# frasermince/gym-cellular-automata

Measured on AMD Instinct MI355X. Metric: cell-updates/sec, 4096x(256x256) ForestFireBulldozer (Alexandridis CA), per-GPU batch, higher is better.
Workload: dtype u8 cells / i16 ages / f32 probabilities

## Files before the change

gym-cellular-automata_amd/csrc/gca_alex_march.hip:

```cpp
#include "gca_alex_rule.h"

#include <type_traits>

#ifndef GCA_MARCH_FLAT_OCC
#define GCA_MARCH_FLAT_OCC 4
#endif
#ifndef GCA_MARCH_OBS_FLAT_OCC
#define GCA_MARCH_OBS_FLAT_OCC 3
#endif
#ifndef GCA_MARCH_XROW
#define GCA_MARCH_XROW 1
#endif

namespace {

constexpr int MW = 256;
constexpr int SH = 16;

struct MarchObs {
    const float4* col;
    const int32_t* night;
    float* rgb;
    const int32_t* action;
    int action_stride, n_choices;
    uint32_t mode_bits;
    uint8_t* refit;
};
constexpr uint32_t OBS_GRID = 0u, OBS_ZERO = 1u, OBS_NONE = 2u;
constexpr uint32_t OBS_CHK_GRID = 4u, OBS_CHK_BLUR = 8u;

__device__ __forceinline__ uint32_t from_prev(uint32_t v) {
    return (uint32_t)__builtin_amdgcn_mov_dpp((int)v, 0x138, 0xF, 0xF, true);
}
__device__ __forceinline__ uint32_t from_next(uint32_t v) {
    return (uint32_t)__builtin_amdgcn_mov_dpp((int)v, 0x130, 0xF, 0xF, true);
}
__device__ __forceinline__ uint32_t from_prev_or(uint32_t old, uint32_t v) {
    return (uint32_t)__builtin_amdgcn_update_dpp((int)old, (int)v, 0x138, 0xF, 0xF, false);
}
__device__ __forceinline__ uint32_t from_next_or(uint32_t old, uint32_t v) {
    return (uint32_t)__builtin_amdgcn_update_dpp((int)old, (int)v, 0x130, 0xF, 0xF, false);
}

template <int J> __device__ __forceinline__ uint64_t byte_lanes(uint32_t x) {
    static_assert(J >= 0 && J < 4, "byte 0..3");
    uint64_t m;
    const uint32_t zero = 0u;
    if constexpr (J == 0) asm("v_cmp_ne_u32_sdwa %0, %1, %2 src0_sel:BYTE_0 src1_sel:DWORD" : "=s"(m) : "v"(x), "s"(zero));
    if constexpr (J == 1) asm("v_cmp_ne_u32_sdwa %0, %1, %2 src0_sel:BYTE_1 src1_sel:DWORD" : "=s"(m) : "v"(x), "s"(zero));
    if constexpr (J == 2) asm("v_cmp_ne_u32_sdwa %0, %1, %2 src0_sel:BYTE_2 src1_sel:DWORD" : "=s"(m) : "v"(x), "s"(zero));
    if constexpr (J == 3) asm("v_cmp_ne_u32_sdwa %0, %1, %2 src0_sel:BYTE_3 src1_sel:DWORD" : "=s"(m) : "v"(x), "s"(zero));
    return m;
}
__device__ __forceinline__ uint32_t lanes_select(uint32_t c, uint64_t m) {
    uint32_t o;
    asm("v_cndmask_b32_e64 %0, 0, %1, %2" : "=v"(o) : "v"(c), "s"(m));
    return o;
}

__host__ __device__ constexpr uint32_t win_mask(int o, int j, int k) {
    uint32_t m = 0;
    for (int b = 0; b < 4; ++b) {
        const int c = 4 * o + b - j;
        if (c >= -k && c <= k) m |= 1u << (8 * b);
    }
    return m;
}
__host__ __device__ constexpr bool win_full(int o, int j, int k) { return j - k <= 4 * o && 4 * o + 3 <= j + k; }
template <bool HALO = false>
__device__ __forceinline__ void window4(uint32_t X, int k, uint32_t (&B)[4], uint32_t z = 0u, uint32_t h1 = 0u,
                                        uint32_t h2 = 0u) {
    uint32_t n[5] = {0u, 0u, X, 0u, 0u};
    if (k >= 1) {
        n[1] = HALO ? from_prev_or(h1, X) : from_prev(X);
        n[3] = HALO ? from_next_or(h1, X) : from_next(X);
    }
    if (k >= 5) {
        n[0] = HALO ? from_prev_or(h2, n[1]) : from_prev(n[1]);
        n[4] = HALO ? from_next_or(h2, n[3]) : from_next(n[3]);
    }
    constexpr uint32_t ONES = 0x01010101u;
    bool use0 = false, useL = false, useR = false, useLR = false;
#pragma unroll
    for (int j = 0; j < 4; ++j) {
        const bool f0 = win_full(0, j, k), fl = win_full(-1, j, k), fr = win_full(1, j, k);
        if (f0 && fl && fr) useLR = true;
        else if (f0 && fl) useL = true;
        else if (f0 && fr) useR = true;
        else if (f0) use0 = true;
    }
    uint32_t S0 = 0u, SL = 0u, SR = 0u, SLR = 0u;
    if (use0 || useL || useR || useLR) S0 = __builtin_amdgcn_udot4(n[2], ONES, z, false);
    if (useL || useLR) SL = __builtin_amdgcn_udot4(n[1], ONES, S0, false);
    if (useR) SR = __builtin_amdgcn_udot4(n[3], ONES, S0, false);
    if (useLR) SLR = __builtin_amdgcn_udot4(n[3], ONES, SL, false);
#pragma unroll
    for (int j = 0; j < 4; ++j) {
        const bool f0 = win_full(0, j, k), fl = win_full(-1, j, k), fr = win_full(1, j, k);
        const bool run = f0;
        uint32_t acc = !run ? z : (fl && fr) ? SLR : fl ? SL : fr ? SR : S0;
#pragma unroll
        for (int o = -2; o <= 2; ++o) {
            if (run && (o == 0 || (o == -1 && fl) || (o == 1 && fr))) continue;
            const uint32_t m = win_mask(o, j, k);
            if (m) acc = __builtin_amdgcn_udot4(n[o + 2], m, acc, false);
        }
        B[j] = acc;
    }
}

__device__ __forceinline__ float4 ldf4(const float* p) { return *reinterpret_cast<const float4*>(p); }
__device__ __forceinline__ gca_f2 m_recip(float v0, float v1) {
    const gca_f2 x = {v0, v1};
    const gca_f2 r0 = {__builtin_amdgcn_rcpf(v0), __builtin_amdgcn_rcpf(v1)};
    const gca_f2 ee = __builtin_elementwise_fma(-x, r0, (gca_f2){1.0f, 1.0f});
    return __builtin_elementwise_fma(ee, r0, r0);
}
__device__ __forceinline__ void m_edge_both(float v0, float v1, gca_f2& own, gca_f2& nb) {
    const gca_f2 rc = m_recip(v0, v1);
    asm("v_max_f32_e64 %0, %1, -%2" : "=v"(own.x) : "v"(v0), "v"(rc.x));
    asm("v_max_f32_e64 %0, %1, -%2" : "=v"(own.y) : "v"(v1), "v"(rc.y));
    asm("v_max_f32_e64 %0, -%1, %2" : "=v"(nb.x) : "v"(v0), "v"(rc.x));
    asm("v_max_f32_e64 %0, -%1, %2" : "=v"(nb.y) : "v"(v1), "v"(rc.y));
}
__device__ __forceinline__ void m_edge_both4(const float4& v, gca_f2& oa, gca_f2& na, gca_f2& ob, gca_f2& nb) {
    const gca_f2 x0 = {v.x, v.y}, x1 = {v.z, v.w};
    const gca_f2 r0 = {__builtin_amdgcn_rcpf(v.x), __builtin_amdgcn_rcpf(v.y)};
    const gca_f2 r1 = {__builtin_amdgcn_rcpf(v.z), __builtin_amdgcn_rcpf(v.w)};
    const gca_f2 e0 = __builtin_elementwise_fma(-x0, r0, (gca_f2){1.0f, 1.0f});
    const gca_f2 e1 = __builtin_elementwise_fma(-x1, r1, (gca_f2){1.0f, 1.0f});
    const gca_f2 c0 = __builtin_elementwise_fma(e0, r0, r0);
    const gca_f2 c1 = __builtin_elementwise_fma(e1, r1, r1);
    asm("v_max_f32_e64 %0, %1, -%2" : "=v"(oa.x) : "v"(v.x), "v"(c0.x));
    asm("v_max_f32_e64 %0, %1, -%2" : "=v"(oa.y) : "v"(v.y), "v"(c0.y));
    asm("v_max_f32_e64 %0, %1, -%2" : "=v"(ob.x) : "v"(v.z), "v"(c1.x));
    asm("v_max_f32_e64 %0, %1, -%2" : "=v"(ob.y) : "v"(v.w), "v"(c1.y));
    asm("v_max_f32_e64 %0, -%1, %2" : "=v"(na.x) : "v"(v.x), "v"(c0.x));
    asm("v_max_f32_e64 %0, -%1, %2" : "=v"(na.y) : "v"(v.y), "v"(c0.y));
    asm("v_max_f32_e64 %0, -%1, %2" : "=v"(nb.x) : "v"(v.z), "v"(c1.x));
    asm("v_max_f32_e64 %0, -%1, %2" : "=v"(nb.y) : "v"(v.w), "v"(c1.y));
}
__device__ __forceinline__ void m_edge_own4(const float4& v, gca_f2& oa, gca_f2& ob) {
    const gca_f2 x0 = {v.x, v.y}, x1 = {v.z, v.w};
    const gca_f2 r0 = {__builtin_amdgcn_rcpf(v.x), __builtin_amdgcn_rcpf(v.y)};
    const gca_f2 r1 = {__builtin_amdgcn_rcpf(v.z), __builtin_amdgcn_rcpf(v.w)};
    const gca_f2 e0 = __builtin_elementwise_fma(-x0, r0, (gca_f2){1.0f, 1.0f});
    const gca_f2 e1 = __builtin_elementwise_fma(-x1, r1, (gca_f2){1.0f, 1.0f});
    const gca_f2 c0 = __builtin_elementwise_fma(e0, r0, r0);
    const gca_f2 c1 = __builtin_elementwise_fma(e1, r1, r1);
    asm("v_max_f32_e64 %0, %1, -%2" : "=v"(oa.x) : "v"(v.x), "v"(c0.x));
    asm("v_max_f32_e64 %0, %1, -%2" : "=v"(oa.y) : "v"(v.y), "v"(c0.y));
    asm("v_max_f32_e64 %0, %1, -%2" : "=v"(ob.x) : "v"(v.z), "v"(c1.x));
    asm("v_max_f32_e64 %0, %1, -%2" : "=v"(ob.y) : "v"(v.w), "v"(c1.y));
}
template <class T, class B> __device__ __forceinline__ T ld_at(const B* base, uint32_t off) {
    return *reinterpret_cast<const T*>(reinterpret_cast<const unsigned char*>(base) + off);
}
template <class T, class B> __device__ __forceinline__ T ld_nt(const B* base, uint32_t off) {
    constexpr int N = (int)(sizeof(T) / 4);
    typedef uint32_t vt __attribute__((ext_vector_type(N)));
    typedef const __attribute__((address_space(1))) unsigned char gbyte;
    typedef const __attribute__((address_space(1))) vt gvt;
    const vt v = __builtin_nontemporal_load((gvt*)((gbyte*)base + off));
    return __builtin_bit_cast(T, v);
}
constexpr uint32_t WZ = 0x4B000000u;
__device__ __forceinline__ gca_f2 wsum_f2(uint32_t b0, uint32_t b1) {
    return (gca_f2){__uint_as_float(b0), __uint_as_float(b1)} - (gca_f2){8388608.0f, 8388608.0f};
}
typedef uint16_t u16x2 __attribute__((ext_vector_type(2)));
typedef int16_t i16x2 __attribute__((ext_vector_type(2)));
__device__ __forceinline__ i16x2 bitcast_i16x2(uint32_t v) { return __builtin_bit_cast(i16x2, v); }
__device__ __forceinline__ u16x2 bitcast_u16x2(uint32_t v) { return __builtin_bit_cast(u16x2, v); }
template <class T> __device__ __forceinline__ uint32_t bitcast_u32(T v) { return __builtin_bit_cast(uint32_t, v); }

constexpr int XI = 16;
constexpr int XS_ONE = 13, XS_TWO = 14;

template <int R, bool OBS, bool GROW, int NSEG, int FLATM>
__global__ __launch_bounds__(NSEG == 1 ? 256 : 64 * NSEG) __attribute__((amdgpu_waves_per_eu(OBS ? (FLATM ? GCA_MARCH_OBS_FLAT_OCC : 2) : (FLATM ? GCA_MARCH_FLAT_OCC : 3), OBS ? (FLATM ? GCA_MARCH_OBS_FLAT_OCC : 2) : (FLATM ? GCA_MARCH_FLAT_OCC : 3)))) void alex_march_kernel(
    gca_alex_params p, int H, int nwaves, const uint8_t* __restrict__ grid_in, uint8_t* __restrict__ grid_out,
    const int16_t* age_in, int16_t* age_out,
    const uint8_t* __restrict__ vd, const uint16_t* __restrict__ dbits, const float* __restrict__ es,
    const int32_t* __restrict__ wind_index, const uint32_t* __restrict__ rng_step, int32_t* __restrict__ counts,
    const uint8_t* __restrict__ act_in, uint8_t* __restrict__ act_out, MarchObs obs) {
    constexpr int NF = 2 * R + 1;
    constexpr int RB = R;
    constexpr bool HALO = NSEG > 1;
    constexpr bool SMASK = !HALO && !OBS && FLATM >= 1;
    constexpr int WPB = HALO ? NSEG : 4;
    constexpr int W = MW * NSEG;
    __shared__ float lut[WPB][16];
    __shared__ float4 colw[WPB][8];
    __shared__ float4 img[OBS ? WPB : 1][OBS ? 192 : 1];
    __shared__ uint32_t fring[WPB][2 * NF * 64];
    __shared__ uint32_t xch[HALO ? 2 : 1][HALO ? NSEG + 2 : 1][4][HALO ? XI : 1];
    __shared__ uint32_t qfl[HALO ? NSEG : 1];
    constexpr bool FLAT = FLATM >= 1, UNI = FLATM == 2;
    constexpr bool XROW = GCA_MARCH_XROW && !HALO && OBS && !FLAT;
    __shared__ float4 xrow[XROW ? 4 : 1][3][XROW ? 64 : 1];
    __shared__ uint32_t xok[XROW ? 4 : 1];

    const int tid = threadIdx.x, wl = __builtin_amdgcn_readfirstlane(tid >> 6), lane = tid & 63;
    const int nb = (int)gridDim.x;
    const int xcd = (int)blockIdx.x & 7, slot = (int)blockIdx.x >> 3;
    const int qn8 = nb >> 3, rn8 = nb & 7;
    const int lb = (xcd < rn8 ? xcd * (qn8 + 1) : rn8 * (qn8 + 1) + (xcd - rn8) * qn8) + slot;
    int strips, e, s, g;
    if constexpr (!HALO) {
        const int wv = lb * 4 + wl;
        if (wv >= nwaves) {
            if constexpr (XROW) {
                if (lane == 0) xok[wl] = 0u;
                __builtin_amdgcn_fence(__ATOMIC_RELEASE, "workgroup", "local");
                __builtin_amdgcn_s_barrier();
            }
            return;
        }
        strips = H / SH;
        e = wv / strips;
        s = wv - e * strips;
        g = 0;
    } else {
        if (lb * NSEG >= nwaves) return;
        strips = H / SH;
        e = lb / strips;
        s = lb - e * strips;
        g = wl;
    }
    const int s0 = s * SH;
    const uint32_t HW = (uint32_t)H * W;
    const uint8_t* gE = grid_in + (size_t)e * HW;
    uint8_t* gO = grid_out + (size_t)e * HW;
    const int16_t* aE = age_in + (size_t)e * HW;
    int16_t* aO = age_out + (size_t)e * HW;
    const uint8_t* vE = UNI ? vd : vd + (size_t)e * HW;
    const uint16_t* dE = dbits + (size_t)e * (HW >> 4);
    const float* sE = FLAT ? es : es + (size_t)e * 4 * HW;
    const uint32_t lc = HALO ? (uint32_t)(MW * g) + 4u * (uint32_t)lane : 4u * (uint32_t)lane;
    const uint32_t ld16 = HALO ? lc >> 4 : (uint32_t)(lane >> 2);
    const uint32_t lane_a = 2u * lc, lane_s = 4u * lc, lane_d = 2u * ld16;
    const uint32_t Fp = rep4((uint32_t)p.fire), Ep = rep4((uint32_t)p.empty), Tp = rep4((uint32_t)p.tree);

    if (lane < 16) lut[wl][lane] = gca_alex_lut_entry(p, lane);
    if (OBS && lane < 6) colw[wl][lane] = obs.col[6 * (obs.night[e] != 0 ? 1 : 0) + lane];
    uint32_t omode = 0u;
    if constexpr (OBS && !HALO) {
        if (obs.action) {
            const int choice = min(max(obs.action[(size_t)e * obs.action_stride + 2], 0), obs.n_choices - 1);
            omode = (uint32_t)__builtin_amdgcn_readfirstlane((int)((obs.mode_bits >> (4 * choice)) & 0xFu));
        }
    }
    auto row0_refit = [&](uint32_t x0, uint32_t x1) -> uint8_t {
        const uint32_t odd = ((x0 + 0x7D7D7D7Du) | x0 | (x1 + 0x7D7D7D7Du) | x1) & 0x80808080u;
        bool pos = false;
        if (omode & OBS_CHK_GRID) pos |= __ballot(x0 != 0u) != 0ull;
        if (omode & OBS_CHK_BLUR) {
            auto hsum = [&](uint32_t x) {
                uint32_t L = __builtin_amdgcn_alignbyte(x, from_prev(x), 3);
                uint32_t Rt = __builtin_amdgcn_alignbyte(from_next(x), x, 1);
                if (lane == 0) L = (x << 8) | (x & 0xFFu);
                if (lane == 63) Rt = (x >> 8) | (x & 0xFF000000u);
                return L + x + Rt;
            };
            const uint32_t S = 2u * hsum(x0) + hsum(x1);
            pos |= __ballot(((S + 0x7B7B7B7Bu) & 0x80808080u) != 0u) != 0ull;
        }
        const bool bad = __ballot(odd != 0u) != 0ull;
        return ((omode & 3u) == OBS_NONE || bad || ((omode & (OBS_CHK_GRID | OBS_CHK_BLUR)) && !pos)) ? 1 : 0;
    };
    __builtin_amdgcn_fence(__ATOMIC_RELEASE, "wavefront");
    __builtin_amdgcn_wave_barrier();
// ... 158 lines not shown
        if constexpr (FLAT) {
            sc[k] = sn[k] = make_float4(1.0f, 1.0f, 1.0f, 1.0f);
        } else {
            sc[k] = ldf4(sE + (size_t)k * HW + (size_t)s0 * W + lc);
            sn[k] = ldf4(sE + (size_t)k * HW + (size_t)min(s0 + 1, H - 1) * W + lc);
        }
    }
    __builtin_amdgcn_fence(__ATOMIC_RELEASE, "wavefront");
    __builtin_amdgcn_wave_barrier();
    __builtin_amdgcn_fence(__ATOMIC_ACQUIRE, "wavefront");
    xrow_publish(true, sc);
    const bool xuse = XROW && wl < 3 && s0 + SH < H && xok[XROW ? wl + 1 : 0] != 0u;
    uint32_t V[R + 1] = {};
    uint32_t Dv1 = 0u, Dv2 = 0u;

    const bool col_lo = lane == 0 && (!HALO || g == 0), col_hi = lane == 63 && (!HALO || g == NSEG - 1);
    const uint32_t xo1 = HALO ? (lane == 63 ? (uint32_t)(((g + 2) * 4 + 0) * XI) : (uint32_t)((g * 4 + 3) * XI)) : 0u;
    const uint32_t xo2 = HALO ? (lane == 63 ? (uint32_t)(((g + 2) * 4 + 1) * XI) : (uint32_t)((g * 4 + 2) * XI)) : 0u;
    auto prep_own = [&](float4& v) {
        gca_f2 a, b;
        m_edge_own4(v, a, b);
        v = make_float4(col_lo ? 1.0f : a.x, a.y, b.x, col_hi ? 1.0f : b.y);
    };
    if constexpr (!FLAT) {
#pragma unroll
        for (int k = 0; k < 3; ++k) prep_own(sc[k]);
    }

    constexpr int NHW = (R + 2) / 2;
    gca_f2 windp[4], hdwp[NHW];
    {
        const int widx = wind_index[e];
#pragma unroll
        for (int q = 0; q < 4; ++q) {
            const int d0 = 2 * q, d1 = 2 * q + 1;
            windp[q] = (gca_f2){p.winds[widx][d0 < 4 ? d0 : d0 + 1], p.winds[widx][d1 < 4 ? d1 : d1 + 1]};
            asm volatile("" : "+v"(windp[q]));
        }
#pragma unroll
        for (int q = 0; q < NHW; ++q) {
            hdwp[q] = (gca_f2){p.heat_dw[2 * q], 2 * q + 1 <= R ? p.heat_dw[2 * q + 1] : 0.0f};
            asm volatile("" : "+v"(hdwp[q]));
        }
    }
    gca_f2 avd = {1.0f, 1.0f};
    if constexpr (UNI) {
        const int b = p.vd_uniform & 0xFF;
        avd = (gca_f2){gca_alex_lut_entry(p, b & 7), gca_alex_lut_entry(p, 8 + ((b >> 4) & 7))};
        asm volatile("" : "+v"(avd));
    }
    auto bcast = [](gca_f2 v, int h) -> gca_f2 {
        return h ? __builtin_shufflevector(v, v, 1, 1) : __builtin_shufflevector(v, v, 0, 0);
    };
    const uint32_t step = rng_step ? rng_step[e] : 0u;
    const uint32_t k0 = (uint32_t)p.seed, k1 = (uint32_t)(p.seed >> 32);
    const uint32_t env_id = (uint32_t)(p.env_offset + e);
    constexpr uint32_t PM0 = 0xD2511F53u, PM1 = 0xCD9E8D57u, PW0 = 0x9E3779B9u, PW1 = 0xBB67AE85u;
    const uint64_t pq1 = (uint64_t)PM1 * step;
    const uint32_t pu0 = (uint32_t)(pq1 >> 32) ^ env_id ^ k0;
    const uint64_t pq2 = (uint64_t)PM0 * pu0;
    const uint32_t pkc = (uint32_t)GCA_TAG_ALEX_CELL ^ k1;
    const uint32_t pkc_age = (uint32_t)GCA_TAG_ALEX_AGE ^ k1;
    const uint32_t pka = (uint32_t)pq1 ^ (k0 + PW0);
    const uint32_t pkb = (uint32_t)(pq2 >> 32) ^ (k1 + PW1);
    const uint32_t pl2 = (uint32_t)pq2;
    auto philox_cell = [&](uint32_t x0, uint32_t rk0, uint32_t rk1, uint32_t ktag) -> u32x4 {
        const uint64_t p0 = (uint64_t)PM0 * x0;
        const uint32_t hi0 = (uint32_t)(p0 >> 32), lo0 = (uint32_t)p0;
        const uint64_t p1 = (uint64_t)PM1 * (hi0 ^ ktag);
        u32x4 c = u32x4{(uint32_t)(p1 >> 32) ^ pka, (uint32_t)p1, lo0 ^ pkb, pl2};
#pragma unroll
        for (int i = 2; i < 10; ++i) {
            const uint64_t a = (uint64_t)PM0 * c.x;
            const uint64_t b = (uint64_t)PM1 * c.z;
            const uint32_t n0 = __builtin_amdgcn_bitop3_b32((uint32_t)(b >> 32), c.y, rk0 + (uint32_t)i * PW0, 0x96);
            const uint32_t n2 = __builtin_amdgcn_bitop3_b32((uint32_t)(a >> 32), c.w, rk1 + (uint32_t)i * PW1, 0x96);
            c = u32x4{n0, (uint32_t)b, n2, (uint32_t)a};
        }
        return c;
    };
    const float pt24 = __fmul_rn(p.p_tree, 16777216.0f);
    const float w_in_minus_bd = __fsub_rn(p.dous_inner, p.dous_border);
    const uint32_t codes = (p.empty & 0xFFu) | ((p.tree & 0xFFu) << 8) | ((p.fire & 0xFFu) << 16);
    int cntE = 0, cntT = 0, cntF = 0;
    uint64_t mP[4] = {}, mC[4] = {};
    if constexpr (SMASK) {
        const uint32_t fa = bytes_eq01(g_init[RB - 1], Fp), fb = bytes_eq01(g_init[RB], Fp);
        mP[0] = byte_lanes<0>(fa); mP[1] = byte_lanes<1>(fa); mP[2] = byte_lanes<2>(fa); mP[3] = byte_lanes<3>(fa);
        mC[0] = byte_lanes<0>(fb); mC[1] = byte_lanes<1>(fb); mC[2] = byte_lanes<2>(fb); mC[3] = byte_lanes<3>(fb);
    }
    uint32_t out_row0 = 0u;

    auto row = [&](const int i, float4 (&SC)[4], float4 (&SN)[4], auto parity) {
        const int r = s0 + i;
        const uint32_t gnew = nG, dnew = nD, own = nOwn, vdw = nVD;
        const uint2 agep = nAge;
        {
            const int rg = r + 1 + R, rd = r + 3;
            const uint32_t r1 = (uint32_t)min(r + 1, H - 1);
            const uint32_t gl = ld_at<uint32_t>(gE + (size_t)min(rg, H - 1) * W, lc);
            const uint32_t d = ld_at<uint16_t>(dE + (size_t)min(rd, H - 1) * (W / 16), lane_d);
            nOwn = ld_at<uint32_t>(gE + (size_t)r1 * W, lc);
            if constexpr (!UNI) nVD = ld_nt<uint32_t>(vE + (size_t)r1 * W, lc);
            nAge = ld_nt<uint2>(aE + (size_t)r1 * W, lane_a);
            nG = rg < H ? gl : Ep;
            nD = rd < H ? d : 0u;
        }
        bool need_next = i + 1 < SH;
        auto load_next_slopes = [&]() {
            if constexpr (XROW) {
                if (i == SH - 2 && xuse) {
#pragma unroll
                    for (int k = 0; k < 3; ++k) SC[k] = xrow[wl + 1][k][lane];
                    SC[3] = SC[2];
                    return;
                }
            }
            const bool need3 = need_next && i + 2 < SH;
            const float* sb = need_next ? sE : es;
            const float* sb3 = need3 ? sE : es;
            const uint32_t rs = need_next ? (uint32_t)min(r + 2, H - 1) : 0u;
            const uint32_t rs3 = need3 ? rs : 0u;
#pragma unroll
            for (int k = 0; k < 4; ++k)
                SC[k] = ld_nt<float4>((k == 3 ? sb3 : sb) + (size_t)k * HW + (size_t)(k == 3 ? rs3 : rs) * W, lane_s);
        };
        uint32_t* Fb = FR + (NF - 1 - (uint32_t)i % NF) * 64;
        {
            const uint32_t fnew = bytes_eq01(gnew, Fp);
            Fb[lane] = fnew;
            Fb[NF * 64 + lane] = fnew;
        }
        __builtin_amdgcn_fence(__ATOMIC_RELEASE, "wavefront");
        __builtin_amdgcn_wave_barrier();
        __builtin_amdgcn_fence(__ATOMIC_ACQUIRE, "wavefront");
        uint32_t fm1, f0, fp1;
        {
            uint32_t rw[NF];
#pragma unroll
            for (int t = 0; t < NF; ++t) rw[t] = Fb[(NF - 1 - t) * 64 + lane];
            V[1] = rw[RB - 1] + rw[RB] + rw[RB + 1];
#pragma unroll
            for (int k = 2; k <= R; ++k) V[k] = V[k - 1] + rw[RB + k] + rw[RB - k];
            fm1 = rw[RB - 1];
            f0 = rw[RB];
            fp1 = rw[RB + 1];
            if constexpr (R >= 3)
                need_next = need_next && __ballot((rw[RB] | rw[RB + 1] | rw[RB + 2] | rw[RB + 3]) != 0u) != 0ull;
        }
        dring[ND - 1] = dflags(dnew);
        Dv1 = dring[1] + dring[2] + dring[3];
        Dv2 = Dv1 + dring[0] + dring[4];
        uint64_t mN[4] = {};
        auto next_lanes = [&]() {
            if constexpr (SMASK) {
                mN[0] = byte_lanes<0>(fp1);
                mN[1] = byte_lanes<1>(fp1);
                mN[2] = byte_lanes<2>(fp1);
                mN[3] = byte_lanes<3>(fp1);
            }
        };

        const uint32_t* xr = nullptr;
        const uint32_t* xr2 = nullptr;
        uint32_t hfm1 = 0u, hf0 = 0u, hfp1 = 0u;
        if constexpr (HALO) {
            constexpr int PAR = decltype(parity)::value;
            if (lane < 2 || lane >= 62) {
                const int xl = lane < 2 ? lane : lane - 60;
                uint4* xd = reinterpret_cast<uint4*>(&xch[PAR][g + 1][xl][0]);
                uint32_t vv[8];
#pragma unroll
                for (int k = 0; k < 8; ++k) vv[k] = k + 1 <= R ? V[k + 1] : 0u;
                const uint32_t sA = lane < 32 ? __float_as_uint(SC[3].x) : __float_as_uint(SN[2].w);
                xd[0] = make_uint4(vv[0], vv[1], vv[2], vv[3]);
                xd[1] = make_uint4(vv[4], vv[5], vv[6], vv[7]);
                xd[2] = make_uint4(Dv1, Dv2, fm1, f0);
                xd[3] = make_uint4(fp1, sA, __float_as_uint(SN[0].x), 0u);
            }
            __builtin_amdgcn_fence(__ATOMIC_RELEASE, "workgroup", "local");
            __builtin_amdgcn_s_barrier();
            __builtin_amdgcn_fence(__ATOMIC_ACQUIRE, "workgroup", "local");
            xr = &xch[PAR][0][0][0] + xo1;
            xr2 = &xch[PAR][0][0][0] + xo2;
            hfm1 = xr[10];
            hf0 = xr[11];
            hfp1 = xr[12];
        }

        const uint32_t treeB = gca_eq_nib(own, Tp), emptyB = gca_eq_nib(own, Ep);
        auto shl_c = [](uint32_t x, uint32_t h) {
            return __builtin_amdgcn_alignbyte(x, HALO ? from_prev_or(h, x) : from_prev(x), 3);
        };
        auto shr_c = [](uint32_t x, uint32_t h) {
            return __builtin_amdgcn_alignbyte(HALO ? from_next_or(h, x) : from_next(x), x, 1);
        };
        auto dir_mask = [&](int d) -> uint32_t {
            const uint32_t row = d < 3 ? fm1 : (d < 5 ? f0 : fp1);
            const uint32_t hrow = d < 3 ? hfm1 : (d < 5 ? hf0 : hfp1);
            const int dc = d < 3 ? d - 1 : (d == 3 ? -1 : (d == 4 ? 1 : d - 6));
            uint32_t m = dc < 0 ? shl_c(row, hrow) : (dc > 0 ? shr_c(row, hrow) : row);
            m *= 0xFFu;
            asm volatile("" : "+v"(m));
            return m;
        };
        auto dir_lanes = [&](int d, int j) -> uint64_t {
            const uint64_t* m = d < 3 ? mP : (d < 5 ? mC : mN);
            const int dc = d < 3 ? d - 1 : (d == 3 ? -1 : (d == 4 ? 1 : d - 6));
            if (dc < 0) return j > 0 ? m[j - 1] : m[3] << 1;
            if (dc > 0) return j < 3 ? m[j + 1] : m[0] >> 1;
            return m[j];
        };
        const uint32_t fireB = (f0 * 0x01020408u) >> 24;
        const uint32_t vor = fm1 | f0 | fp1, hvor = hfm1 | hf0 | hfp1;
        const uint32_t anyfire = (((vor | shl_c(vor, hvor) | shr_c(vor, hvor)) & 0x01010101u) * 0x01020408u) >> 24;
        gca_f2 qn[2] = {{1.0f, 1.0f}, {1.0f, 1.0f}};
        const bool row_need = __ballot((treeB & anyfire) != 0u) != 0ull;
        const bool kill_row = r == 0 || r == H - 1;
        const bool kill_next = r + 1 == H - 1;
        auto prep_next = [&](int k, bool want_nb, float (&nbv)[4]) {
            gca_f2 oa, ob, na, nb2;
            if (want_nb) {
                m_edge_both4(SN[k], oa, na, ob, nb2);
                nbv[0] = na.x; nbv[1] = na.y; nbv[2] = nb2.x; nbv[3] = nb2.y;
            } else {
                m_edge_own4(SN[k], oa, ob);
            }
            SN[k] = make_float4(col_lo ? 1.0f : oa.x, oa.y, ob.x, col_hi ? 1.0f : ob.y);
        };
        if (!row_need) {
            next_lanes();
            if constexpr (!FLAT) {
                load_next_slopes();
                float unused[4];
#pragma unroll
                for (int k = 0; k < 3; ++k) prep_next(k, false, unused);
            }
        } else {
            gca_f2 ph[2] = {{p.heat0, p.heat0}, {p.heat0, p.heat0}};
#pragma unroll
            for (int k = 0; k <= R; ++k) {
                uint32_t B[4];
                if (k == 0) {
#pragma unroll
                    for (int j = 0; j < 4; ++j) B[j] = (f0 >> (8 * j)) & 0xFFu;
                } else {
                    if constexpr (HALO)
                        window4<true>(V[k], k, B, WZ, xr[k - 1], k >= 5 ? xr2[k - 1] : 0u);
                    else
                        window4(V[k], k, B, WZ);
                }
                gca_f2 bs[2];
#pragma unroll
                for (int h = 0; h < 2; ++h)
                    bs[h] = k == 0 ? (gca_f2){(float)B[2 * h], (float)B[2 * h + 1]} : wsum_f2(B[2 * h], B[2 * h + 1]);
#pragma unroll
                for (int h = 0; h < 2; ++h) ph[h] = __builtin_elementwise_fma(bcast(hdwp[k >> 1], k & 1), bs[h], ph[h]);
                asm volatile("" : "+v"(ph[0]), "+v"(ph[1]));
                __builtin_amdgcn_sched_barrier(0);
            }
            const bool dous_any = __ballot((Dv2 | (HALO ? xr[8] | xr[9] : 0u)) != 0u) != 0ull;
            if (dous_any) {
                uint32_t D1[4], D2[4];
                if constexpr (HALO) {
                    window4<true>(Dv1, 1, D1, WZ, xr[8]);
                    window4<true>(Dv2, 2, D2, WZ, xr[9]);
                } else {
                    window4(Dv1, 1, D1, WZ);
                    window4(Dv2, 2, D2, WZ);
                }
                gca_f2 d1[2], d2[2], dz[2];
#pragma unroll
                for (int h = 0; h < 2; ++h) d1[h] = wsum_f2(D1[2 * h], D1[2 * h + 1]);
#pragma unroll
                for (int h = 0; h < 2; ++h) d2[h] = wsum_f2(D2[2 * h], D2[2 * h + 1]);
#pragma unroll
                for (int h = 0; h < 2; ++h) dz[h] = (gca_f2){w_in_minus_bd, w_in_minus_bd} * d1[h];
#pragma unroll
                for (int h = 0; h < 2; ++h)
                    dz[h] = __builtin_elementwise_fma((gca_f2){p.dous_border, p.dous_border}, d2[h], dz[h]);
#pragma unroll
                for (int h = 0; h < 2; ++h) ph[h] = ph[h] - dz[h];
            }
            if constexpr (UNI) {
#pragma unroll
                for (int h = 0; h < 2; ++h) ph[h] = ph[h] * bcast(avd, 0);
#pragma unroll
                for (int h = 0; h < 2; ++h) ph[h] = ph[h] * bcast(avd, 1);
            } else {
                gca_f2 av[2], ad[2];
#pragma unroll
                for (int h = 0; h < 2; ++h) {
                    const uint32_t b0 = (vdw >> (16 * h)) & 0xFFu, b1 = (vdw >> (16 * h + 8)) & 0xFFu;
                    av[h] = (gca_f2){lut[wl][b0 & 7u], lut[wl][b1 & 7u]};
                    ad[h] = (gca_f2){lut[wl][8 + (b0 >> 4)], lut[wl][8 + (b1 >> 4)]};
                }
#pragma unroll
                for (int h = 0; h < 2; ++h) ph[h] = ph[h] * av[h];
#pragma unroll
                for (int h = 0; h < 2; ++h) ph[h] = ph[h] * ad[h];
// ... 23 lines not shown
                        }
                    } else {
                        const uint32_t Md = dir_mask(d);
#pragma unroll
                        for (int h = 0; h < 2; ++h) {
                            cm[h][0] = __float_as_uint(c[h].x) & (uint32_t)(int32_t)(int8_t)(Md >> (16 * h));
                            cm[h][1] = __float_as_uint(c[h].y) & (uint32_t)(int32_t)(int8_t)(Md >> (16 * h + 8));
                        }
                    }
#pragma unroll
                    for (int h = 0; h < 2; ++h)
                        qn[h] = __builtin_elementwise_fma(-qn[h], (gca_f2){__uint_as_float(cm[h][0]), __uint_as_float(cm[h][1])},
                                                          qn[h]);
                    __builtin_amdgcn_sched_barrier(0);
                };
                const float one[4] = {1.0f, 1.0f, 1.0f, 1.0f};
                uint32_t h45 = 0x3F800000u, h7 = 0x3F800000u;
                if constexpr (HALO && !KILL) {
                    gca_f2 o_, n_;
                    m_edge_both(__uint_as_float(xr[XS_ONE]), __uint_as_float(xr[XS_TWO]), o_, n_);
                    h45 = __float_as_uint(n_.x);
                    h7 = __float_as_uint(n_.y);
                }
#pragma unroll
                for (int d = 0; d < 3; ++d) {
                    const float a[4] = {SC[d].x, SC[d].y, SC[d].z, SC[d].w};
                    apply(d, KILL ? one : a);
                }
                if (KILL) {
                    apply(3, one);
                    apply(4, one);
                } else {
                    gca_f2 oa, ob, na, nb2;
                    m_edge_both4(SC[3], oa, na, ob, nb2);
                    const float a3[4] = {col_lo ? 1.0f : oa.x, oa.y, ob.x, col_hi ? 1.0f : ob.y};
                    apply(3, a3);
                    const float nx = __uint_as_float((uint32_t)__builtin_amdgcn_update_dpp(
                        (int)h45, (int)__float_as_uint(na.x), 0x130, 0xF, 0xF, false));
                    const float a4[4] = {col_lo ? 1.0f : na.y, nb2.x, nb2.y, nx};
                    apply(4, a4);
                }
                if constexpr (!FLAT) load_next_slopes();
                next_lanes();
                float nb[4];
                if constexpr (!FLAT) prep_next(2, !KILL, nb);
                if (KILL) {
                    apply(5, one);
                } else {
                    const float pv = __uint_as_float((uint32_t)__builtin_amdgcn_update_dpp(
                        (int)h45, (int)__float_as_uint(nb[3]), 0x138, 0xF, 0xF, false));
                    const float a5[4] = {pv, nb[0], nb[1], col_hi ? 1.0f : nb[2]};
                    apply(5, a5);
                }
                if constexpr (!FLAT) prep_next(1, !KILL, nb);
                if (KILL) {
                    apply(6, one);
                } else {
                    const float a6[4] = {col_lo ? 1.0f : nb[0], nb[1], nb[2], col_hi ? 1.0f : nb[3]};
                    apply(6, a6);
                }
                if constexpr (!FLAT) prep_next(0, !KILL, nb);
                if (KILL) {
                    apply(7, one);
                } else {
                    const float nx = __uint_as_float((uint32_t)__builtin_amdgcn_update_dpp(
                        (int)h7, (int)__float_as_uint(nb[0]), 0x130, 0xF, 0xF, false));
                    const float a7[4] = {col_lo ? 1.0f : nb[1], nb[2], nb[3], nx};
                    apply(7, a7);
                }
            };
            if (FLAT || kill_row)
                dir_pass(std::true_type{});
            else
                dir_pass(std::false_type{});
        }
        if (kill_next) {
#pragma unroll
            for (int k = 0; k < 3; ++k) SN[k] = make_float4(1.0f, 1.0f, 1.0f, 1.0f);
        }

        const uint32_t needB = (treeB & anyfire) | (GROW ? emptyB : 0u);
        const uint32_t lin0 = (uint32_t)r * W + lc;
        uint32_t burn = 0u, grow = 0u, NA[2];
        const bool wave_draws = __ballot(needB != 0u) != 0ull;
        uint32_t rk0 = k0, rk1 = k1;
        asm volatile("" : "+s"(rk0), "+s"(rk1));
        u32x4 X = u32x4{0u, 0u, 0u, 0u};
        if (wave_draws) X = philox_cell(lin0 >> 2, rk0, rk1, pkc);
        const uint32_t xw[4] = {X.x, X.y, X.z, X.w};
#pragma unroll
        for (int h = 0; h < 2; ++h) {
            const gca_f2 thr = __builtin_elementwise_fma(qn[h], (gca_f2){-16777216.0f, -16777216.0f},
                                                         (gca_f2){16777216.0f, 16777216.0f});
            const float u0 = (float)(xw[2 * h] >> 8), u1 = (float)(xw[2 * h + 1] >> 8);
            burn |= (u0 < thr.x ? 1u : 0u) << (2 * h);
            burn |= (u1 < thr.y ? 1u : 0u) << (2 * h + 1);
            if constexpr (GROW) {
                grow |= (u0 < pt24 ? 1u : 0u) << (2 * h);
                grow |= (u1 < pt24 ? 1u : 0u) << (2 * h + 1);
            }
        }
        burn &= treeB;
        grow &= emptyB;
        {
            const uint32_t spare = __builtin_amdgcn_perm(__builtin_amdgcn_perm(X.w, X.z, 0x0c0c0400u),
                                                         __builtin_amdgcn_perm(X.y, X.x, 0x0c0c0400u), 0x05040100u);
            const uint32_t n0 = (uint32_t)randint_ms(spare, p.age_lo, p.age_hi);
            NA[0] = NA[1] = __builtin_amdgcn_perm(n0, n0, 0x05040100u);
            if (__ballot((burn & (burn - 1u)) != 0u) != 0ull) {
                const u32x4 Y = philox_cell(lin0 >> 2, rk0, rk1, pkc_age);
                const uint32_t nk[4] = {n0, (uint32_t)randint_ms(Y.x, p.age_lo, p.age_hi),
                                        (uint32_t)randint_ms(Y.y, p.age_lo, p.age_hi),
                                        (uint32_t)randint_ms(Y.z, p.age_lo, p.age_hi)};
                uint32_t a[4];
#pragma unroll
                for (int j = 0; j < 4; ++j) {
                    const uint32_t rank = (uint32_t)__builtin_popcount(burn & ((1u << j) - 1u));
                    a[j] = rank == 0 ? nk[0] : (rank == 1 ? nk[1] : (rank == 2 ? nk[2] : nk[3]));
                }
                NA[0] = __builtin_amdgcn_perm(a[1], a[0], 0x05040100u);
                NA[1] = __builtin_amdgcn_perm(a[3], a[2], 0x05040100u);
            }
        }

        const uint32_t agw[2] = {agep.x, agep.y};
        uint32_t le1;
        if (!p.burnout_eq1) {
            const uint32_t y0 = bitcast_u32(__builtin_elementwise_sub_sat(bitcast_i16x2(agw[0]), (i16x2){2, 2}));
            const uint32_t y1 = bitcast_u32(__builtin_elementwise_sub_sat(bitcast_i16x2(agw[1]), (i16x2){2, 2}));
            le1 = ((y0 >> 15) & 1u) | ((y0 >> 30) & 2u) | ((y1 >> 13) & 4u) | ((y1 >> 28) & 8u);
        } else {
            le1 = 0u;
#pragma unroll
            for (int j = 0; j < 4; ++j)
                le1 |= ((int32_t)(int16_t)(agw[j >> 1] >> (16 * (j & 1))) == 1) ? (1u << j) : 0u;
        }
        const uint32_t newF = burn | (fireB & ~le1);
        const uint32_t newT = (treeB & ~burn) | grow;
        const uint32_t newE = (emptyB & ~grow) | (fireB & le1);
        const uint32_t keepB = ~(treeB | emptyB | fireB) & 0xFu;
        uint32_t sel = gca_spread4(newT) + 2u * gca_spread4(newF);
        sel |= (gca_spread4(keepB) * 0xFFu) & 0x07060504u;
        const uint32_t outw = __builtin_amdgcn_perm(own, codes, sel);
        uint32_t nag[2];
#pragma unroll
        for (int h = 0; h < 2; ++h) {
            const uint32_t fh = ((fireB >> (2 * h)) & 1u) | (((fireB >> (2 * h + 1)) & 1u) << 16);
            const uint32_t a1 = bitcast_u32(bitcast_u16x2(agw[h]) - bitcast_u16x2(fh));
            const uint32_t bm = (((burn >> (2 * h)) & 1u) * 0xFFFFu) | (((burn >> (2 * h + 1)) & 1u) * 0xFFFF0000u);
            nag[h] = gca_bfi32(bm, NA[h], a1);
        }
        const size_t o = (size_t)r * W + lc;
        __builtin_nontemporal_store(outw, reinterpret_cast<uint32_t*>(gO + o));
        { typedef uint32_t u2v __attribute__((ext_vector_type(2)));
          __builtin_nontemporal_store((u2v){nag[0], nag[1]}, reinterpret_cast<u2v*>(aO + o)); }
        write_rgb_row(r, newT, newF, dring[DB]);
        if constexpr (OBS && !HALO) {
            if (obs.refit && r < 2) {
                if (r == 0) {
                    out_row0 = outw;
                } else {
                    const uint8_t rf = row0_refit(out_row0, outw);
                    if (lane == 0) obs.refit[e] = rf;
                }
            }
        }
        cntT += __builtin_popcount(newT);
        cntF += __builtin_popcount(newF);
        cntE += __builtin_popcount(newE);

#pragma unroll
        for (int t = 0; t < ND - 1; ++t) dring[t] = dring[t + 1];
        if constexpr (SMASK) {
#pragma unroll
            for (int j = 0; j < 4; ++j) {
                mP[j] = mC[j];
                mC[j] = mN[j];
            }
        }
    };
#pragma unroll 1
    for (int i = 0; i < SH; i += 2) {
        row(i, sc, sn, std::integral_constant<int, 0>{});
        row(i + 1, sn, sc, std::integral_constant<int, 1>{});
    }

    if (counts || act_out) {
        const bool anyF = __ballot(cntF != 0) != 0ull;
        if (act_out && lane == 0) act_out[((size_t)e * strips + s) * NSEG + g] = anyF ? 1 : 0;
        if (counts) {
#pragma unroll
            for (int off = 32; off > 0; off >>= 1) {
                cntT += __shfl_xor(cntT, off);
                cntF += __shfl_xor(cntF, off);
                cntE += __shfl_xor(cntE, off);
            }
            if (lane == 0) {
                if (cntE) atomicAdd(counts + 3 * e + 0, cntE);
                if (cntT) atomicAdd(counts + 3 * e + 1, cntT);
                if (cntF) atomicAdd(counts + 3 * e + 2, cntF);
            }
        }
    }
}

template <int R, bool OBS, bool GROW, int NSEG, int FLATM>
void launch_march_n(const gca_alex_params& p, int E, int H, const uint8_t* gi, uint8_t* go, const int16_t* ai,
                    int16_t* ao, const uint8_t* vd, const uint16_t* db, const float* es, const int32_t* wi,
                    const uint32_t* rs, int32_t* counts, const uint8_t* act_in, uint8_t* act_out, MarchObs obs,
                    hipStream_t st) {
    const int nwaves = E * (H / SH) * NSEG;
    if constexpr (NSEG == 1)
        hipLaunchKernelGGL((alex_march_kernel<R, OBS, GROW, 1, FLATM>), dim3((unsigned)((nwaves + 3) / 4)), dim3(256), 0, st, p,
                           H, nwaves, gi, go, ai, ao, vd, db, es, wi, rs, counts, act_in, act_out, obs);
    else
        hipLaunchKernelGGL((alex_march_kernel<R, OBS, GROW, NSEG, FLATM>), dim3((unsigned)(nwaves / NSEG)), dim3(64 * NSEG), 0,
                           st, p, H, nwaves, gi, go, ai, ao, vd, db, es, wi, rs, counts, act_in, act_out, obs);
}
template <int R, bool OBS, bool GROW, int FLATM>
void launch_march_g(const gca_alex_params& p, int E, int H, int W, const uint8_t* gi, uint8_t* go, const int16_t* ai,
                    int16_t* ao, const uint8_t* vd, const uint16_t* db, const float* es, const int32_t* wi,
                    const uint32_t* rs, int32_t* counts, const uint8_t* act_in, uint8_t* act_out, MarchObs obs,
                    hipStream_t st) {
    if (W == MW)
        launch_march_n<R, OBS, GROW, 1, FLATM>(p, E, H, gi, go, ai, ao, vd, db, es, wi, rs, counts, act_in, act_out, obs, st);
    else if (W == 2 * MW)
        launch_march_n<R, OBS, GROW, 2, FLATM>(p, E, H, gi, go, ai, ao, vd, db, es, wi, rs, counts, act_in, act_out, obs, st);
    else
        launch_march_n<R, OBS, GROW, 4, FLATM>(p, E, H, gi, go, ai, ao, vd, db, es, wi, rs, counts, act_in, act_out, obs, st);
}
template <int R, bool OBS>
void launch_march(const gca_alex_params& p, int E, int H, int W, const uint8_t* gi, uint8_t* go, const int16_t* ai,
                  int16_t* ao, const uint8_t* vd, const uint16_t* db, const float* es, const int32_t* wi,
                  const uint32_t* rs, int32_t* counts, const uint8_t* act_in, uint8_t* act_out, MarchObs obs,
                  hipStream_t st) {
    const bool grow = p.p_tree > 0.0f;
    const int fm = es ? 0 : (vd ? 1 : 2);
#define GCA_MARCH_FM(FM)                                                                                                \
    if (grow)                                                                                                         \
        launch_march_g<R, OBS, true, FM>(p, E, H, W, gi, go, ai, ao, vd, db, es, wi, rs, counts, act_in, act_out, obs, st); \
    else                                                                                                              \
        launch_march_g<R, OBS, false, FM>(p, E, H, W, gi, go, ai, ao, vd, db, es, wi, rs, counts, act_in, act_out, obs, st);
    if (fm == 0) {
        GCA_MARCH_FM(0)
    } else if (fm == 1) {
        GCA_MARCH_FM(1)
    } else {
        GCA_MARCH_FM(2)
    }
#undef GCA_MARCH_FM
}

template <bool OBS>
void dispatch_march(const gca_alex_params& p, int E, int H, int W, const uint8_t* gi, uint8_t* go, const int16_t* ai,
                    int16_t* ao, const uint8_t* vd, const uint16_t* db, const float* es, const int32_t* wi,
                    const uint32_t* rs, int32_t* counts, const uint8_t* act_in, uint8_t* act_out, MarchObs obs,
                    hipStream_t st) {
#define GCA_MARCH_CASE(RV) \
    case RV: launch_march<RV, OBS>(p, E, H, W, gi, go, ai, ao, vd, db, es, wi, rs, counts, act_in, act_out, obs, st); break;
    switch (p.R) {
#ifdef GCA_MARCH_ANALYSIS_R6
        GCA_MARCH_CASE(6)
#else
        GCA_MARCH_CASE(1) GCA_MARCH_CASE(2) GCA_MARCH_CASE(3) GCA_MARCH_CASE(4)
        GCA_MARCH_CASE(5) GCA_MARCH_CASE(6) GCA_MARCH_CASE(7) GCA_MARCH_CASE(8)
#endif
    }
#undef GCA_MARCH_CASE
}

int march_impl(const gca_alex_params* p, int E, int H, int W, const uint8_t* grid_in, uint8_t* grid_out,
               const int16_t* age_in, int16_t* age_out, const uint8_t* vd, const uint16_t* dous_bits,
               const float* edge_slope, const int32_t* wind_index, const uint32_t* rng_step, int32_t* counts,
               const uint8_t* act_in, uint8_t* act_out, MarchObs obs, void* stream) {
    GCA_CHECK_ARG(p && grid_in && grid_out && age_in && age_out && dous_bits && wind_index,
                  "alex_step_march: null argument");
    GCA_CHECK_ARG(vd || (!edge_slope && p->vd_uniform >= 0 && p->vd_uniform <= 255 && (p->vd_uniform & 0x88) == 0),
                  "alex_step_march: vd = NULL (uniform layers) needs edge_slope = NULL and p->vd_uniform = "
// ... 101 lines not shown
```

Before: 1243 billion.

## Compute march cell updates as wave-wide lane masks with SDWA byte writes

For the flat, no-observation, no-growth march variant, per-cell state and age updates are rebuilt around 64-bit lane masks: ballots over random draws, SDWA compares of cell bytes and ages, and SDWA cndmask byte/word writes into the output words. Counts come from popcounts of wave-uniform masks, so the final shuffle reduction is skipped. The aim is to drop the per-lane nibble/perm bookkeeping and reduction work. In exchange it relies on inline asm that clobbers VCC and adds scalar mask work per byte, which could raise SALU pressure or serialise.

```diff
diff --git a/gym-cellular-automata_amd/csrc/gca_alex_march.hip b/gym-cellular-automata_amd/csrc/gca_alex_march.hip
--- a/gym-cellular-automata_amd/csrc/gca_alex_march.hip
+++ b/gym-cellular-automata_amd/csrc/gca_alex_march.hip
@@ -56,6 +56,69 @@
     uint32_t o;
     asm("v_cndmask_b32_e64 %0, 0, %1, %2" : "=v"(o) : "v"(c), "s"(m));
     return o;
+}
+
+#define GCA_SDWA_J(J, TEXT, SEL0, SEL1, SEL2, SEL3, TAIL, ...)        \
+    if constexpr ((J) == 0) asm(TEXT SEL0 TAIL __VA_ARGS__);         \
+    if constexpr ((J) == 1) asm(TEXT SEL1 TAIL __VA_ARGS__);         \
+    if constexpr ((J) == 2) asm(TEXT SEL2 TAIL __VA_ARGS__);         \
+    if constexpr ((J) == 3) asm(TEXT SEL3 TAIL __VA_ARGS__)
+template <int J, int K> __device__ __forceinline__ uint64_t byte_eq_lanes(uint32_t x, uint32_t c) {
+    static_assert(K >= 0 && K < 2, "byte 0..1 of the codes");
+    uint64_t m;
+#define GCA_BYTE_EQ(KS)                                                                                         \
+    GCA_SDWA_J(J, "v_cmp_eq_u32_sdwa %0, %1, %2 src0_sel:", "BYTE_0", "BYTE_1", "BYTE_2", "BYTE_3", " src1_sel:" KS, \
+               : "=s"(m) : "v"(x), "v"(c))
+    if constexpr (K == 0) { GCA_BYTE_EQ("BYTE_0"); }
+    if constexpr (K == 1) { GCA_BYTE_EQ("BYTE_1"); }
+#undef GCA_BYTE_EQ
+    return m;
+}
+template <int J> __device__ __forceinline__ uint64_t age_lt_lanes(uint32_t x, uint32_t c) {
+    uint64_t m;
+    GCA_SDWA_J(J & 1, "v_cmp_lt_i32_sdwa %0, sext(%1), sext(%2) src0_sel:", "WORD_0", "WORD_1", "WORD_0", "WORD_1",
+               " src1_sel:WORD_0", : "=s"(m) : "v"(x), "v"(c));
+    return m;
+}
+template <int J> __device__ __forceinline__ uint64_t age_eq_lanes(uint32_t x, uint32_t c) {
+    uint64_t m;
+    GCA_SDWA_J(J & 1, "v_cmp_eq_i32_sdwa %0, sext(%1), sext(%2) src0_sel:", "WORD_0", "WORD_1", "WORD_0", "WORD_1",
+               " src1_sel:WORD_1", : "=s"(m) : "v"(x), "v"(c));
+    return m;
+}
+template <int J, int K> __device__ __forceinline__ void put_byte(uint32_t& out, uint32_t src, uint64_t m) {
+    static_assert(K >= 0 && K < 3, "byte 0..2 of the codes");
+#define GCA_PUT_BYTE(KS)                                                                                      \
+    GCA_SDWA_J(J, "s_mov_b64 vcc, %2\n\tv_cndmask_b32_sdwa %0, %0, %1, vcc ",                                   \
+               "dst_sel:BYTE_0 dst_unused:UNUSED_PRESERVE src0_sel:BYTE_0",                                   \
+               "dst_sel:BYTE_1 dst_unused:UNUSED_PRESERVE src0_sel:BYTE_1",                                   \
+               "dst_sel:BYTE_2 dst_unused:UNUSED_PRESERVE src0_sel:BYTE_2",                                   \
+               "dst_sel:BYTE_3 dst_unused:UNUSED_PRESERVE src0_sel:BYTE_3", " src1_sel:" KS,                  \
+               : "+v"(out) : "v"(src), "s"(m) : "vcc")
+    if constexpr (K == 0) { GCA_PUT_BYTE("BYTE_0"); }
+    if constexpr (K == 1) { GCA_PUT_BYTE("BYTE_1"); }
+    if constexpr (K == 2) { GCA_PUT_BYTE("BYTE_2"); }
+#undef GCA_PUT_BYTE
+}
+template <int J, int K> __device__ __forceinline__ void put_age(uint32_t& w, uint32_t src, uint64_t m) {
+    static_assert(K >= 0 && K < 2, "int16 0..1 of the source");
+#define GCA_PUT_AGE(KS)                                                                                       \
+    GCA_SDWA_J(J & 1, "s_mov_b64 vcc, %2\n\tv_cndmask_b32_sdwa %0, %0, %1, vcc ",                               \
+               "dst_sel:WORD_0 dst_unused:UNUSED_PRESERVE src0_sel:WORD_0",                                   \
+               "dst_sel:WORD_1 dst_unused:UNUSED_PRESERVE src0_sel:WORD_1",                                   \
+               "dst_sel:WORD_0 dst_unused:UNUSED_PRESERVE src0_sel:WORD_0",                                   \
+               "dst_sel:WORD_1 dst_unused:UNUSED_PRESERVE src0_sel:WORD_1", " src1_sel:" KS,                  \
+               : "+v"(w) : "v"(src), "s"(m) : "vcc")
+    if constexpr (K == 0) { GCA_PUT_AGE("WORD_0"); }
+    if constexpr (K == 1) { GCA_PUT_AGE("WORD_1"); }
+#undef GCA_PUT_AGE
+}
+#undef GCA_SDWA_J
+template <class F> __device__ __forceinline__ void for4(F&& f) {
+    f(std::integral_constant<int, 0>{});
+    f(std::integral_constant<int, 1>{});
+    f(std::integral_constant<int, 2>{});
+    f(std::integral_constant<int, 3>{});
 }
 
 __host__ __device__ constexpr uint32_t win_mask(int o, int j, int k) {
@@ -188,6 +251,7 @@
     constexpr int RB = R;
     constexpr bool HALO = NSEG > 1;
     constexpr bool SMASK = !HALO && !OBS && FLATM >= 1;
+    constexpr bool RMASK = SMASK && !GROW;
     constexpr int WPB = HALO ? NSEG : 4;
     constexpr int W = MW * NSEG;
     __shared__ float lut[WPB][16];
@@ -512,6 +576,8 @@
     const float pt24 = __fmul_rn(p.p_tree, 16777216.0f);
     const float w_in_minus_bd = __fsub_rn(p.dous_inner, p.dous_border);
     const uint32_t codes = (p.empty & 0xFFu) | ((p.tree & 0xFFu) << 8) | ((p.fire & 0xFFu) << 16);
+    uint32_t codesv = codes, agekv = 0x00010002u;
+    asm volatile("" : "+v"(codesv), "+v"(agekv));
     int cntE = 0, cntT = 0, cntF = 0;
     uint64_t mP[4] = {}, mC[4] = {};
     if constexpr (SMASK) {
@@ -618,7 +684,7 @@
             hfp1 = xr[12];
         }
 
-        const uint32_t treeB = gca_eq_nib(own, Tp), emptyB = gca_eq_nib(own, Ep);
+        const uint32_t treeB = RMASK ? 0u : gca_eq_nib(own, Tp), emptyB = RMASK ? 0u : gca_eq_nib(own, Ep);
         auto shl_c = [](uint32_t x, uint32_t h) {
             return __builtin_amdgcn_alignbyte(x, HALO ? from_prev_or(h, x) : from_prev(x), 3);
         };
@@ -641,11 +707,17 @@
             if (dc > 0) return j < 3 ? m[j + 1] : m[0] >> 1;
             return m[j];
         };
-        const uint32_t fireB = (f0 * 0x01020408u) >> 24;
-        const uint32_t vor = fm1 | f0 | fp1, hvor = hfm1 | hf0 | hfp1;
-        const uint32_t anyfire = (((vor | shl_c(vor, hvor) | shr_c(vor, hvor)) & 0x01010101u) * 0x01020408u) >> 24;
+        uint32_t fireB = 0u, anyfire = 0u;
+        bool row_need;
+        if constexpr (RMASK) {
+            row_need = __ballot(V[1] != 0u) != 0ull;
+        } else {
+            fireB = (f0 * 0x01020408u) >> 24;
+            const uint32_t vor = fm1 | f0 | fp1, hvor = hfm1 | hf0 | hfp1;
+            anyfire = (((vor | shl_c(vor, hvor) | shr_c(vor, hvor)) & 0x01010101u) * 0x01020408u) >> 24;
+            row_need = __ballot((treeB & anyfire) != 0u) != 0ull;
+        }
         gca_f2 qn[2] = {{1.0f, 1.0f}, {1.0f, 1.0f}};
-        const bool row_need = __ballot((treeB & anyfire) != 0u) != 0ull;
         const bool kill_row = r == 0 || r == H - 1;
         const bool kill_next = r + 1 == H - 1;
         auto prep_next = [&](int k, bool want_nb, float (&nbv)[4]) {
@@ -835,32 +907,55 @@
         const uint32_t needB = (treeB & anyfire) | (GROW ? emptyB : 0u);
         const uint32_t lin0 = (uint32_t)r * W + lc;
         uint32_t burn = 0u, grow = 0u, NA[2];
-        const bool wave_draws = __ballot(needB != 0u) != 0ull;
+        const bool wave_draws = RMASK ? row_need : __ballot(needB != 0u) != 0ull;
         uint32_t rk0 = k0, rk1 = k1;
         asm volatile("" : "+s"(rk0), "+s"(rk1));
         u32x4 X = u32x4{0u, 0u, 0u, 0u};
         if (wave_draws) X = philox_cell(lin0 >> 2, rk0, rk1, pkc);
         const uint32_t xw[4] = {X.x, X.y, X.z, X.w};
+        uint64_t bL[4] = {};
+        uint32_t NAv[4] = {};
+        gca_f2 thr[2];
+        float u[4];
 #pragma unroll
         for (int h = 0; h < 2; ++h) {
-            const gca_f2 thr = __builtin_elementwise_fma(qn[h], (gca_f2){-16777216.0f, -16777216.0f},
-                                                         (gca_f2){16777216.0f, 16777216.0f});
-            const float u0 = (float)(xw[2 * h] >> 8), u1 = (float)(xw[2 * h + 1] >> 8);
-            burn |= (u0 < thr.x ? 1u : 0u) << (2 * h);
-            burn |= (u1 < thr.y ? 1u : 0u) << (2 * h + 1);
-            if constexpr (GROW) {
-                grow |= (u0 < pt24 ? 1u : 0u) << (2 * h);
-                grow |= (u1 < pt24 ? 1u : 0u) << (2 * h + 1);
-            }
-        }
-        burn &= treeB;
-        grow &= emptyB;
+            thr[h] = __builtin_elementwise_fma(qn[h], (gca_f2){-16777216.0f, -16777216.0f},
+                                               (gca_f2){16777216.0f, 16777216.0f});
+            u[2 * h] = (float)(xw[2 * h] >> 8);
+            u[2 * h + 1] = (float)(xw[2 * h + 1] >> 8);
+        }
+        if constexpr (RMASK) {
+            for4([&](auto jc) {
+                constexpr int j = decltype(jc)::value;
+                const uint64_t mT = byte_eq_lanes<j, 1>(own, codesv);
+                bL[j] = __ballot(u[j] < ((j & 1) ? thr[j >> 1].y : thr[j >> 1].x)) & mT;
+                cntT += __builtin_popcountll(mT & ~bL[j]);
+            });
+        } else {
+#pragma unroll
+            for (int j = 0; j < 4; ++j) {
+                burn |= (u[j] < ((j & 1) ? thr[j >> 1].y : thr[j >> 1].x) ? 1u : 0u) << j;
+                if constexpr (GROW) grow |= (u[j] < pt24 ? 1u : 0u) << j;
+            }
+            burn &= treeB;
+            grow &= emptyB;
+        }
         {
             const uint32_t spare = __builtin_amdgcn_perm(__builtin_amdgcn_perm(X.w, X.z, 0x0c0c0400u),
                                                          __builtin_amdgcn_perm(X.y, X.x, 0x0c0c0400u), 0x05040100u);
             const uint32_t n0 = (uint32_t)randint_ms(spare, p.age_lo, p.age_hi);
-            NA[0] = NA[1] = __builtin_amdgcn_perm(n0, n0, 0x05040100u);
-            if (__ballot((burn & (burn - 1u)) != 0u) != 0ull) {
+            bool multi;
+            if constexpr (RMASK) {
+                NAv[0] = NAv[1] = NAv[2] = NAv[3] = n0;
+                const uint64_t b01 = bL[0] | bL[1];
+                multi = ((bL[0] & bL[1]) | (b01 & bL[2]) | ((b01 | bL[2]) & bL[3])) != 0ull;
+            } else {
+                NA[0] = NA[1] = __builtin_amdgcn_perm(n0, n0, 0x05040100u);
+                multi = __ballot((burn & (burn - 1u)) != 0u) != 0ull;
+            }
+            if (multi) {
+                if constexpr (RMASK)
+                    burn = lanes_select(1u, bL[0]) | lanes_select(2u, bL[1]) | lanes_select(4u, bL[2]);
                 const u32x4 Y = philox_cell(lin0 >> 2, rk0, rk1, pkc_age);
                 const uint32_t nk[4] = {n0, (uint32_t)randint_ms(Y.x, p.age_lo, p.age_hi),
                                         (uint32_t)randint_ms(Y.y, p.age_lo, p.age_hi),
@@ -871,37 +966,74 @@
                     const uint32_t rank = (uint32_t)__builtin_popcount(burn & ((1u << j) - 1u));
                     a[j] = rank == 0 ? nk[0] : (rank == 1 ? nk[1] : (rank == 2 ? nk[2] : nk[3]));
                 }
-                NA[0] = __builtin_amdgcn_perm(a[1], a[0], 0x05040100u);
-                NA[1] = __builtin_amdgcn_perm(a[3], a[2], 0x05040100u);
+                if constexpr (RMASK) {
+#pragma unroll
+                    for (int j = 0; j < 4; ++j) NAv[j] = a[j];
+                } else {
+                    NA[0] = __builtin_amdgcn_perm(a[1], a[0], 0x05040100u);
+                    NA[1] = __builtin_amdgcn_perm(a[3], a[2], 0x05040100u);
+                }
             }
         }
 
         const uint32_t agw[2] = {agep.x, agep.y};
-        uint32_t le1;
-        if (!p.burnout_eq1) {
-            const uint32_t y0 = bitcast_u32(__builtin_elementwise_sub_sat(bitcast_i16x2(agw[0]), (i16x2){2, 2}));
-            const uint32_t y1 = bitcast_u32(__builtin_elementwise_sub_sat(bitcast_i16x2(agw[1]), (i16x2){2, 2}));
-            le1 = ((y0 >> 15) & 1u) | ((y0 >> 30) & 2u) | ((y1 >> 13) & 4u) | ((y1 >> 28) & 8u);
+        uint32_t outw, nag[2], newT = 0u, newF = 0u;
+        if constexpr (RMASK) {
+            uint32_t dec[2];
+#pragma unroll
+            for (int h = 0; h < 2; ++h) dec[h] = bitcast_u32(bitcast_u16x2(agw[h]) - (u16x2){1, 1});
+            outw = own;
+            nag[0] = agw[0];
+            nag[1] = agw[1];
+            auto cells = [&](auto eq1) {
+              for4([&](auto jc) {
+                constexpr int j = decltype(jc)::value;
+                const uint64_t le = decltype(eq1)::value ? age_eq_lanes<j>(agw[j >> 1], agekv) : age_lt_lanes<j>(agw[j >> 1], agekv);
+                const uint64_t fire = mC[j], out = fire & le;
+                const uint64_t mEj = byte_eq_lanes<j, 0>(own, codesv);
+                cntF += __builtin_popcountll(bL[j] | (fire & ~le));
+                cntE += __builtin_popcountll(mEj | out);
+                put_byte<j, 2>(outw, codesv, bL[j]);
+                put_byte<j, 0>(outw, codesv, out);
+                put_age<j, j & 1>(nag[j >> 1], dec[j >> 1], fire);
+                put_age<j, 0>(nag[j >> 1], NAv[j], bL[j]);
+              });
+            };
+            int eq1 = p.burnout_eq1;
+            asm volatile("" : "+s"(eq1));
+            if (!eq1)
+                cells(std::false_type{});
+            else
+                cells(std::true_type{});
         } else {
-            le1 = 0u;
-#pragma unroll
-            for (int j = 0; j < 4; ++j)
-                le1 |= ((int32_t)(int16_t)(agw[j >> 1] >> (16 * (j & 1))) == 1) ? (1u << j) : 0u;
-        }
-        const uint32_t newF = burn | (fireB & ~le1);
-        const uint32_t newT = (treeB & ~burn) | grow;
-        const uint32_t newE = (emptyB & ~grow) | (fireB & le1);
-        const uint32_t keepB = ~(treeB | emptyB | fireB) & 0xFu;
-        uint32_t sel = gca_spread4(newT) + 2u * gca_spread4(newF);
-        sel |= (gca_spread4(keepB) * 0xFFu) & 0x07060504u;
-        const uint32_t outw = __builtin_amdgcn_perm(own, codes, sel);
-        uint32_t nag[2];
-#pragma unroll
-        for (int h = 0; h < 2; ++h) {
-            const uint32_t fh = ((fireB >> (2 * h)) & 1u) | (((fireB >> (2 * h + 1)) & 1u) << 16);
-            const uint32_t a1 = bitcast_u32(bitcast_u16x2(agw[h]) - bitcast_u16x2(fh));
-            const uint32_t bm = (((burn >> (2 * h)) & 1u) * 0xFFFFu) | (((burn >> (2 * h + 1)) & 1u) * 0xFFFF0000u);
-            nag[h] = gca_bfi32(bm, NA[h], a1);
+            uint32_t le1;
+            if (!p.burnout_eq1) {
+                const uint32_t y0 = bitcast_u32(__builtin_elementwise_sub_sat(bitcast_i16x2(agw[0]), (i16x2){2, 2}));
+                const uint32_t y1 = bitcast_u32(__builtin_elementwise_sub_sat(bitcast_i16x2(agw[1]), (i16x2){2, 2}));
+                le1 = ((y0 >> 15) & 1u) | ((y0 >> 30) & 2u) | ((y1 >> 13) & 4u) | ((y1 >> 28) & 8u);
+            } else {
+                le1 = 0u;
+#pragma unroll
+                for (int j = 0; j < 4; ++j)
+                    le1 |= ((int32_t)(int16_t)(agw[j >> 1] >> (16 * (j & 1))) == 1) ? (1u << j) : 0u;
+            }
+            newF = burn | (fireB & ~le1);
+            newT = (treeB & ~burn) | grow;
+            const uint32_t newE = (emptyB & ~grow) | (fireB & le1);
+            const uint32_t keepB = ~(treeB | emptyB | fireB) & 0xFu;
+            uint32_t sel = gca_spread4(newT) + 2u * gca_spread4(newF);
+            sel |= (gca_spread4(keepB) * 0xFFu) & 0x07060504u;
+            outw = __builtin_amdgcn_perm(own, codes, sel);
+#pragma unroll
+            for (int h = 0; h < 2; ++h) {
+                const uint32_t fh = ((fireB >> (2 * h)) & 1u) | (((fireB >> (2 * h + 1)) & 1u) << 16);
+                const uint32_t a1 = bitcast_u32(bitcast_u16x2(agw[h]) - bitcast_u16x2(fh));
+                const uint32_t bm = (((burn >> (2 * h)) & 1u) * 0xFFFFu) | (((burn >> (2 * h + 1)) & 1u) * 0xFFFF0000u);
+                nag[h] = gca_bfi32(bm, NA[h], a1);
+            }
+            cntT += __builtin_popcount(newT);
+            cntF += __builtin_popcount(newF);
+            cntE += __builtin_popcount(newE);
         }
         const size_t o = (size_t)r * W + lc;
         __builtin_nontemporal_store(outw, reinterpret_cast<uint32_t*>(gO + o));
@@ -918,10 +1050,6 @@
                 }
             }
         }
-        cntT += __builtin_popcount(newT);
-        cntF += __builtin_popcount(newF);
-        cntE += __builtin_popcount(newE);
-
 #pragma unroll
         for (int t = 0; t < ND - 1; ++t) dring[t] = dring[t + 1];
         if constexpr (SMASK) {
@@ -942,11 +1070,13 @@
         const bool anyF = __ballot(cntF != 0) != 0ull;
         if (act_out && lane == 0) act_out[((size_t)e * strips + s) * NSEG + g] = anyF ? 1 : 0;
         if (counts) {
-#pragma unroll
-            for (int off = 32; off > 0; off >>= 1) {
-                cntT += __shfl_xor(cntT, off);
-                cntF += __shfl_xor(cntF, off);
-                cntE += __shfl_xor(cntE, off);
+            if constexpr (!RMASK) {
+#pragma unroll
+                for (int off = 32; off > 0; off >>= 1) {
+                    cntT += __shfl_xor(cntT, off);
+                    cntF += __shfl_xor(cntF, off);
+                    cntE += __shfl_xor(cntE, off);
+                }
             }
             if (lane == 0) {
                 if (cntE) atomicAdd(counts + 3 * e + 0, cntE);
```

New measurement: 958.1 billion. 22.9% lower.
